# bdina9/qat-vit

Hardware: AMD Instinct MI355X
Metric: images/sec QAT student step (fwd+bwd+allreduce) (higher is better)
Workload: dtype f32 (emulated: int8 MFMA for grid x grid products; forward float operands as fp16 hi+lo pairs; backward gradients as ONE fp16 plane scaled per tensor - 2^-12 per element, <= 4e-4 relative L2 per stage against the fp32 reference, bf16-pair fallback on overflow; fp32 / exact-integer accumulate)

## Files before the change

include/qatvit.h:

```cpp
#ifndef QATVIT_H
#define QATVIT_H

#include <stdint.h>

#ifdef __cplusplus
extern "C" {
#endif
#if defined(__GNUC__) || defined(__clang__)
#pragma GCC visibility push(default)
#endif

#define QATVIT_ABI_VERSION 4

int qatvit_abi_version(void);
const char* qatvit_last_error(void);
const char* qatvit_target_arch(void);

int64_t qatvit_fq_workspace_bytes(int64_t channels);
int qatvit_fq_forward(const float* x, float* y, uint8_t* mask_bits,
                      float* running_min, float* running_max, float* scale, int32_t* zero_point,
                      const int64_t* observer_on, const int64_t* fake_quant_on,
                      float averaging_const, int32_t qmin, int32_t qmax,
                      int64_t channels, int64_t inner, int32_t per_channel, int32_t symmetric,
                      void* workspace, void* stream);
// ... 6 lines not shown
                       const float* rstd, float* dx, float* dgamma, float* dbeta,
                       int64_t rows, int64_t dim, void* stream);

int qatvit_kd_ce_loss(const float* student, const float* teacher, const int64_t* labels,
                      int64_t batch, int64_t classes, float kd_temp, float kd_alpha,
                      float label_smoothing, float* out3, float* dlogits, void* stream);

int qatvit_kd_ce_loss_table(const float* student, const float* table, int64_t table_rows,
                            const int64_t* index, const int64_t* labels, int64_t batch,
                            int64_t classes, float kd_temp, float kd_alpha, float label_smoothing,
                            float* out3, float* dlogits, void* stream);


int qatvit_gemm_nt(const void* A_hi, const void* A_lo, const void* B, float* C, int32_t M, int32_t N, int32_t K,
                   int32_t lda, int32_t ldb, int32_t ldc, const float* s1, const float* s2, const float* col_scale,
                   const float* bias, uint32_t* stats, void* stream);

int qatvit_gemm_nt_f16(const void* A16_hi, const void* A16_lo, const void* B16, float* C, int32_t M, int32_t N, int32_t K, int32_t lda, int32_t ldb,
                       int32_t ldc, const float* s1, const float* s2, const float* col_scale, const float* bias, uint32_t* stats, void* stream);

int qatvit_gemm_nt_i8_minmax(const void* A8, const void* B8, const int32_t* wsum, const float* a_qp, int32_t center, int32_t M, int32_t N, int32_t K,
                             int32_t lda, int32_t ldb, const float* s1, const float* s2, const float* col_scale, const float* bias, uint32_t* stats,
                             void* stream);

int qatvit_w8_fragment_order(const void* B8, void* B8f, int32_t N, int32_t K, void* stream);

int qatvit_i8_strip(int32_t mode, const void* A8, const void* B8f, const int32_t* wsum, const float* a_qp, int32_t center, int32_t M, int32_t N, int32_t K,
                    int32_t lda, const float* s1, const float* s2, const float* col_scale, const float* bias, uint32_t* stats, const float* out_qp,
                    int32_t qmin, int32_t qmax, void* out8, void* out8_mask, int32_t code_T, uint32_t* lut_out, uint32_t* lutq_out,
                    float* out16_scale, void* stream);

int qatvit_ln_apply_quant8(const float* x, const float* mean, const float* rstd, const float* gamma, const float* beta, const float* qp, int32_t qmin, int32_t qmax,
                           void* out8, int32_t center, int64_t M, int32_t D, void* stream);

int qatvit_i8_strip_ln(const float* x, const float* mean, const float* rstd, const float* gamma, const float* beta, int32_t ln_qmin, int32_t ln_qmax, void* out8,
                       const void* B8f, const int32_t* wsum, const float* a_qp, int32_t center, int32_t M, int32_t N, int32_t K, int32_t lda, const float* s2,
                       const float* col_scale, const float* bias, uint32_t* stats, void* stream);

int qatvit_gemm_nt_codes(const void* A8, const uint32_t* lut, const void* B16, float* C, int32_t M, int32_t N, int32_t K, int32_t lda, int32_t ldb,
                         int32_t ldc, const float* s1, const float* s2, const float* col_scale, const float* bias, uint32_t* stats, void* stream);

int qatvit_gemm_nt_i8(const void* A8, const void* B8, const int32_t* wsum, const float* a_qp, int32_t center, float* C, int32_t M,
                      int32_t N, int32_t K, int32_t lda, int32_t ldb, int32_t ldc, const float* s1, const float* s2,
                      const float* col_scale, const float* bias, uint32_t* stats, void* stream);

int64_t qatvit_gemm_tn_scratch_bytes(void);
int qatvit_gemm_tn_codes(const void* P_hi, const void* P_lo, const void* Qc, const uint32_t* lutQ, float* C, int32_t M, int32_t N, int32_t Kw, int32_t ldp,
                         int32_t ldq, int32_t ldc, const float* s1, const float* W, const float* w_scale, const int32_t* w_zp, int32_t w_per_channel,
                         int32_t w_qmin, int32_t w_qmax, float* dbias, const float* row_div, float* scratch, int64_t scratch_bytes, void* stream);
int qatvit_gemm_tn(const void* P_hi, const void* P_lo, const void* Q_hi, const void* Q_lo, float* C, int32_t M, int32_t N,
                   int32_t Kw, int32_t ldp, int32_t ldq, int32_t ldc, const float* s1, const float* W, const float* w_scale,
                   const int32_t* w_zp, int32_t w_per_channel, int32_t w_qmin, int32_t w_qmax, float* dbias,
                   const float* row_div, float* scratch, int64_t scratch_bytes, void* stream);

int qatvit_gemm_nt_dy16(const void* A16, const void* B16, float* C, int32_t M, int32_t N, int32_t K, int32_t lda, int32_t ldb, int32_t ldc, const float* s1,
                        const float* s2, void* stream);
int qatvit_gemm_tn_dy16(const void* P16, const void* Q_hi, const void* Q_lo, const void* Qc, const uint32_t* lutQ16, float* C, int32_t M, int32_t N, int32_t Kw,
                        int32_t ldp, int32_t ldq, int32_t ldc, const float* s1, const float* s2, const float* W, const float* w_scale, const int32_t* w_zp,
                        int32_t w_per_channel, int32_t w_qmin, int32_t w_qmax, float* dbias, const float* row_div, float* scratch, int64_t scratch_bytes,
                        void* stream);
int qatvit_gemm_tn_q8_dy16(const void* P16, const void* Q8, const float* a_qp, int32_t center, float* C, int32_t M, int32_t N, int32_t Kw, int32_t ldp, int32_t ldq,
                           int32_t ldc, const float* s2, const float* W, const float* w_scale, const int32_t* w_zp, int32_t w_per_channel, int32_t w_qmin,
                           int32_t w_qmax, float* dbias, const float* row_div, float* scratch, int64_t scratch_bytes, void* stream);

struct qatvit_tn_item {
    const void* P; const void* Q; const uint32_t* lut; const float* s1; const float* s2; float* C; const float* W; const float* w_scale; const int32_t* w_zp; float* dbias;
// ... 129 lines not shown
```

qat-vit_amd/csrc/capi.hip:

```cpp
#include <stdarg.h>
#include <stdlib.h>
#include <string.h>

#include "../../include/qatvit.h"
#include "qv_common.h"
#include "qv_kernels.h"

namespace qv {
static thread_local char g_err[512] = "";
void set_error(const char* fmt, ...) {
    va_list ap;
    va_start(ap, fmt);
    vsnprintf(g_err, sizeof(g_err), fmt, ap);
    va_end(ap);
}

static bool knob(const char* name) {
    const char* v = getenv(name);
    return !v || atoi(v) != 0;
}
const Knobs& knobs() {
    static const Knobs k{knob("QATVIT_I8"), knob("QATVIT_F16"), knob("QATVIT_FC2_CODES"), knob("QATVIT_FC1_BITS"), knob("QATVIT_FC2W_CODES"),
                         knob("QATVIT_WBATCH"), knob("QATVIT_ATTN_CODES"), knob("QATVIT_QKV_2PASS"), knob("QATVIT_LNB_FUSE"), knob("QATVIT_QP_LATE"),
                         knob("QATVIT_TN_STREAM"), knob("QATVIT_TN_Q8"), knob("QATVIT_ATTN_BWD_FUSED"), knob("QATVIT_F16_STRIP"), knob("QATVIT_I8_STRIP"), knob("QATVIT_LN_STRIP")};
// ... 112 lines not shown
    if (launch_w8_fragment_order(B8, B8f, N, K, (hipStream_t)stream)) return 1;
    QV_CHECK_LAUNCH("qatvit_w8_fragment_order");
    return 0;
}

int qatvit_i8_strip(int32_t mode, const void* A8, const void* B8f, const int32_t* wsum, const float* a_qp, int32_t center, int32_t M, int32_t N, int32_t K,
                    int32_t lda, const float* s1, const float* s2, const float* col_scale, const float* bias, uint32_t* stats, const float* out_qp,
                    int32_t qmin, int32_t qmax, void* out8, void* out8_mask, int32_t code_T, uint32_t* lut_out, uint32_t* lutq_out,
                    float* out16_scale, void* stream) {
    QV_CHECK_ARG(A8 && B8f && wsum && a_qp && s1, "qatvit_i8_strip: null pointer argument");
    QV_CHECK_ARG(mode == 3 || mode == 4 || mode == 7, "qatvit_i8_strip: mode %d (3 = statistics, 7 = qkv codes, 4 = fc1 codes)", mode);
    NTPost post{};
    post.mode = mode;
    post.qp = out_qp; post.qmin = qmin; post.qmax = qmax; post.out8 = out8; post.out8_mask = out8_mask; post.code_T = code_T; post.code_hd = 64;
    post.lut_out = lut_out; post.lutq_out = lutq_out; post.out16_scale = out16_scale;
    if (!launch_i8_strip(A8, B8f, wsum, a_qp, center, M, N, K, lda, N, s1, s2, col_scale, bias, stats, 1, (hipStream_t)stream, &post, true)) {
        set_error("qatvit_i8_strip: unsupported arguments (mode %d M=%d N=%d K=%d lda=%d: need K = 384 with N %% 1152 == 0 or N %% 1536 == 0, or K = 768 with "
                  "N = 2304 or 3072; lda %% 16 == 0, M < 2^22, the mode's output pointers, qmax - qmin < 256; mode 7: (N / 3) %% 384 == 0, 0 < code_T < 1024)",
                  mode, M, N, K, lda);
        return 1;
    }
    QV_CHECK_LAUNCH("qatvit_i8_strip");
    return 0;
}

int qatvit_ln_apply_quant8(const float* x, const float* mean, const float* rstd, const float* gamma, const float* beta, const float* qp, int32_t qmin, int32_t qmax,
                           void* out8, int32_t center, int64_t M, int32_t D, void* stream) {
    QV_CHECK_ARG(x && mean && rstd && gamma && beta && qp && out8, "qatvit_ln_apply_quant8: null pointer argument");
    QV_CHECK_ARG(M >= 1 && D >= 4 && D % 4 == 0, "qatvit_ln_apply_quant8: M=%lld D=%d (D %% 4 == 0)", (long long)M, D);
    if (launch_ln_apply_quant(x, mean, rstd, gamma, beta, qp, qmin, qmax, nullptr, M, D, (hipStream_t)stream, out8, center)) return 1;
    QV_CHECK_LAUNCH("qatvit_ln_apply_quant8");
    return 0;
}

int qatvit_i8_strip_ln(const float* x, const float* mean, const float* rstd, const float* gamma, const float* beta, int32_t ln_qmin, int32_t ln_qmax, void* out8,
                       const void* B8f, const int32_t* wsum, const float* a_qp, int32_t center, int32_t M, int32_t N, int32_t K, int32_t lda, const float* s2,
                       const float* col_scale, const float* bias, uint32_t* stats, void* stream) {
    QV_CHECK_ARG(x && mean && rstd && gamma && beta && out8 && B8f && wsum && a_qp && stats, "qatvit_i8_strip_ln: null pointer argument");
    if (!launch_i8_strip_ln(x, mean, rstd, gamma, beta, ln_qmin, ln_qmax, out8, B8f, wsum, a_qp, center, M, N, K, lda, s2, col_scale, bias, stats, 1,
                            (hipStream_t)stream, true)) {
        set_error("qatvit_i8_strip_ln: unsupported arguments (M=%d N=%d K=%d lda=%d: need K = 384 with N = 1152 or 1536, or K = 768 with N = 2304 or 3072; "
                  "lda %% 16 == 0, lda >= K, 0 < M < 2^22)", M, N, K, lda);
        return 1;
    }
    QV_CHECK_LAUNCH("qatvit_i8_strip_ln");
    return 0;
}

int qatvit_gemm_nt_codes(const void* A8, const uint32_t* lut, const void* B16, float* C, int32_t M, int32_t N, int32_t K, int32_t lda, int32_t ldb,
                         int32_t ldc, const float* s1, const float* s2, const float* col_scale, const float* bias, uint32_t* stats, void* stream) {
    QV_CHECK_ARG(A8 && lut && B16 && C, "qatvit_gemm_nt_codes: null pointer argument");
    if (launch_gemm_nt_codes(A8, lut, B16, C, M, N, K, lda, ldb, ldc, s1, s2, col_scale, bias, stats, 1, (hipStream_t)stream)) return 1;
    QV_CHECK_LAUNCH("qatvit_gemm_nt_codes");
    return 0;
}

int qatvit_gemm_nt_i8(const void* A8, const void* B8, const int32_t* wsum, const float* a_qp, int32_t center, float* C, int32_t M, int32_t N,
                      int32_t K, int32_t lda, int32_t ldb, int32_t ldc, const float* s1, const float* s2, const float* col_scale, const float* bias,
                      uint32_t* stats, void* stream) {
    QV_CHECK_ARG(A8 && B8 && wsum && a_qp && C, "qatvit_gemm_nt_i8: null pointer argument");
    if (launch_gemm_nt_i8(A8, B8, wsum, a_qp, center, C, M, N, K, lda, ldb, ldc, s1, s2, col_scale, bias, stats, 1, (hipStream_t)stream)) return 1;
    QV_CHECK_LAUNCH("qatvit_gemm_nt_i8");
    return 0;
}

int qatvit_gemm_tn(const void* P_hi, const void* P_lo, const void* Q_hi, const void* Q_lo, float* C, int32_t M, int32_t N, int32_t Kw, int32_t ldp,
// ... 153 lines not shown
```

qat-vit_amd/csrc/elt.hip:

```cpp
#include <stdlib.h>

#include "qv_common.h"
#include "qv_device.h"
#include "qv_kernels.h"
#include "qv_qparams.h"

namespace qv {

struct QP { float s, inv, zp, on; };
__device__ inline QP load_qp(const float* qp) { return QP{qp[0], qp[1], qp[2], qp[3]}; }
__device__ inline float fqv(float x, const QP& q, float fqmin, float fqmax, bool& in) {
    const float t = rintf(x * q.inv) + q.zp;
    in = (t >= fqmin && t <= fqmax) || q.on == 0.f;
    const float y = (fminf(fmaxf(t, fqmin), fqmax) - q.zp) * q.s;
    return q.on != 0.f ? y : x;
}
__device__ inline float fqi(float x, const QP& q, float fqmin, float fqmax) {
    return fminf(fmaxf(rintf(x * q.inv) + q.zp, fqmin), fqmax) - q.zp;
}

__device__ inline void store_split4(__bf16* hi, __bf16* lo, int64_t off, float a, float b, float c, float d) {
    uint2 h, l;
    split_pair(a, b, h.x, l.x);
    split_pair(c, d, h.y, l.y);
// ... 106 lines not shown
            if (act[j]) s += (v[j].x + v[j].y) + (v[j].z + v[j].w);
        }
#pragma unroll
        for (int j = 0; j < NV; ++j)
            if (MODE != 2 && act[j]) *reinterpret_cast<float4*>(x_new + row * D + cc[j]) = v[j];
        const float mu = wave_sum(s) / (float)D;
        float qq = 0.f;
#pragma unroll
        for (int j = 0; j < NV; ++j) {
            v[j].x -= mu; v[j].y -= mu; v[j].z -= mu; v[j].w -= mu;
            if (act[j]) qq += (v[j].x * v[j].x + v[j].y * v[j].y) + (v[j].z * v[j].z + v[j].w * v[j].w);
        }
        const float rs = rsqrtf(wave_sum(qq) / (float)D + eps);
        if (lane == 0) { mean[row] = mu; rstd[row] = rs; }
        if (MODE == 1 && maskbits && lane < 4) {
#pragma unroll
            for (int j = 0; j < NV; ++j)
                maskbits[(row * NV + j) * 4 + lane] = lane == 0 ? mb[j][0] : lane == 1 ? mb[j][1] : lane == 2 ? mb[j][2] : mb[j][3];
        }
#pragma unroll
        for (int j = 0; j < NV; ++j) {
            if (act[j]) {
                const float o0 = v[j].x * rs * g[j].x + bb[j].x, o1 = v[j].y * rs * g[j].y + bb[j].y, o2 = v[j].z * rs * g[j].z + bb[j].z,
                            o3 = v[j].w * rs * g[j].w + bb[j].w;
                mn = fminf(fminf(mn, o0), fminf(o1, fminf(o2, o3)));
                mx = fmaxf(fmaxf(mx, o0), fmaxf(o1, fmaxf(o2, o3)));
            }
        }
    }
    mn = wave_min(mn);
    mx = wave_max(mx);
    __shared__ float smn[4], smx[4];
    if (lane == 0) { smn[threadIdx.x >> 6] = mn; smx[threadIdx.x >> 6] = mx; }
    __syncthreads();
    const float bmn = fminf(fminf(smn[0], smn[1]), fminf(smn[2], smn[3])), bmx = fmaxf(fmaxf(smx[0], smx[1]), fmaxf(smx[2], smx[3]));
    if (threadIdx.x == 0) stat_atomic(stats, stat_slots, bmn, bmx);
}

__global__ __launch_bounds__(256) void k_ln_apply_quant(const float* __restrict__ x, const float* __restrict__ mean, const float* __restrict__ rstd,
                                                        const float* __restrict__ gamma, const float* __restrict__ beta, const float* __restrict__ qp,
                                                        int qmin, int qmax, __bf16* __restrict__ out, int64_t M, int D,
                                                        int8_t* __restrict__ out8, int center, int out_f16, const QpLate late) {
    __shared__ float sQp[4];
    QP q;
    if (late.stats) { const float4 r = qp_late_resolve(late, sQp); q = QP{r.x, r.y, r.z, r.w}; }
    else q = load_qp(qp);
    const int d4 = D / 4;
    const int64_t n4 = M * d4;
    for (int64_t i = blockIdx.x * (int64_t)blockDim.x + threadIdx.x; i < n4; i += (int64_t)gridDim.x * blockDim.x) {
        const int64_t row = i / d4;
        const int c = (int)(i % d4) * 4;
        const float mu = mean[row], rs = rstd[row];
        const float4 v = *reinterpret_cast<const float4*>(x + row * D + c);
        const float4 g = *reinterpret_cast<const float4*>(gamma + c), b = *reinterpret_cast<const float4*>(beta + c);
        bf16x4 o;
        o[0] = (__bf16)fqi((v.x - mu) * rs * g.x + b.x, q, qmin, qmax);
        o[1] = (__bf16)fqi((v.y - mu) * rs * g.y + b.y, q, qmin, qmax);
        o[2] = (__bf16)fqi((v.z - mu) * rs * g.z + b.z, q, qmin, qmax);
        o[3] = (__bf16)fqi((v.w - mu) * rs * g.w + b.w, q, qmin, qmax);
        if (out && out_f16) *reinterpret_cast<uint2*>(out + row * D + c) = make_uint2(pk_f16((float)o[0], (float)o[1]), pk_f16((float)o[2], (float)o[3]));
        else if (out) *reinterpret_cast<bf16x4*>(out + row * D + c) = o;
        if (out8) {
            const float sh = q.zp - (float)center;
            char4 o8 = make_char4((signed char)((float)o[0] + sh), (signed char)((float)o[1] + sh), (signed char)((float)o[2] + sh),
                                  (signed char)((float)o[3] + sh));
            *reinterpret_cast<char4*>(out8 + row * D + c) = o8;
// ... 392 lines not shown
__global__ __launch_bounds__(256) void k_wquant(const float* __restrict__ W, const float* __restrict__ qp, int per_channel, int qmin, int qmax,
                                                __bf16* __restrict__ wq, __bf16* __restrict__ wqT, int N, int K) {
    wquant_body(W, qp, per_channel, qmin, qmax, wq, wqT, N, K, blockIdx.x, blockIdx.y);
}
__global__ __launch_bounds__(256) void k_w_quant_all(const WQuantTab t) {
    int wi = 0;
    while (wi + 1 < t.n && (int)blockIdx.x >= t.blk0[wi + 1]) ++wi;
    const int b = blockIdx.x - t.blk0[wi], kt = (t.K[wi] + 31) / 32;
    wquant_body(t.W[wi], t.qp[wi], t.per_channel, t.qmin, t.qmax, reinterpret_cast<__bf16*>(t.wq[wi]), reinterpret_cast<__bf16*>(t.wqT[wi]), t.N[wi],
                t.K[wi], b % kt, b / kt, reinterpret_cast<int8_t*>(t.w8[wi]), t.wsum[wi], reinterpret_cast<_Float16*>(t.w16[wi]),
                reinterpret_cast<int8_t*>(t.w8f[wi]), t.wT16 ? wT16_gap_bytes(t.N[wi], t.K[wi]) : 0, ((t.wT16f_mask >> wi) & 1ull) != 0);
}
static_assert(sizeof(WQuantTab) <= 4096, "WQuantTab travels as a kernel argument");
__global__ __launch_bounds__(256) void k_w8_fragment_order(const int8_t* __restrict__ B8, int8_t* __restrict__ B8f, int N, int K) {
    const int64_t i = blockIdx.x * (int64_t)blockDim.x + threadIdx.x;
    if (i >= (int64_t)N * K) return;
    B8f[w8f_offset((int)(i / K), (int)(i % K), K)] = B8[i];
}
int launch_w8_fragment_order(const void* B8, void* B8f, int N, int K, hipStream_t st) {
    if (N < 48 || N % 48 != 0 || K % 64 != 0 || !B8 || !B8f) { set_error("w8_fragment_order: need N %% 48 == 0, K %% 64 == 0 (N=%d K=%d)", N, K); return 1; }
    k_w8_fragment_order<<<cdiv((int64_t)N * K, 256), 256, 0, st>>>(reinterpret_cast<const int8_t*>(B8), reinterpret_cast<int8_t*>(B8f), N, K);
    return 0;
}

int launch_img_patches(const float* img, void* out_bf16, const float* qp, int qmin, int qmax, int B, int C, int H, int W, int P, hipStream_t st,
                       void* out8, int center) {
    if (P % 8 != 0 || H % P != 0 || W % P != 0) { set_error("img_patches: patch %d must be a multiple of 8 and divide %dx%d", P, H, W); return 1; }
    const int64_t n8 = (int64_t)B * C * H * W / 8;
    k_img_patches<<<flat_grid(n8), 256, 0, st>>>(img, reinterpret_cast<__bf16*>(out_bf16), qp, qmin, qmax, B, C, H, W, P, reinterpret_cast<int8_t*>(out8),
                                                 center);
    return 0;
}

int launch_resid_fq_lnstats(int mode, const float* x_prev, const float* Y, const float* qpY, int qmin, int qmax, const float* cls, const float* pos,
                            float* x_new, float* mean, float* rstd, const float* gamma, const float* beta, float eps, uint32_t* stats, int stat_slots,
                            int64_t M, int D, int T, hipStream_t st, void* maskbits, const QpLate* late) {
    if (D % 4 != 0 || D > 256 * kMaxV) { set_error("resid_fq_lnstats: D=%d unsupported (need D%%4==0, D<=768)", D); return 1; }
    unsigned long long* mbits = mode != 1 ? nullptr : reinterpret_cast<unsigned long long*>(maskbits);
    const QpLate lt = late ? *late : QpLate{};
#define QV_RESID(MODE_, NV_) k_resid_fq_lnstats<MODE_, NV_><<<rows_grid(M), 256, 0, st>>>(x_prev, Y, qpY, qmin, qmax, cls, pos, x_new, mean, rstd, gamma, beta, eps, stats, stat_slots, M, D, T, mbits, lt)
    const int nv = (D + 255) / 256;
    if (mode == 0) { if (nv == 1) QV_RESID(0, 1); else if (nv == 2) QV_RESID(0, 2); else QV_RESID(0, 3); }
    else if (mode == 1) { if (nv == 1) QV_RESID(1, 1); else if (nv == 2) QV_RESID(1, 2); else QV_RESID(1, 3); }
    else { if (nv == 1) QV_RESID(2, 1); else if (nv == 2) QV_RESID(2, 2); else QV_RESID(2, 3); }
#undef QV_RESID
    return 0;
}

int launch_ln_apply_quant(const float* x, const float* mean, const float* rstd, const float* gamma, const float* beta, const float* qp, int qmin,
                          int qmax, void* out_bf16, int64_t M, int D, hipStream_t st, void* out8, int center, bool out_f16, const QpLate* late) {
    k_ln_apply_quant<<<flat_grid(M * (D / 4)), 256, 0, st>>>(x, mean, rstd, gamma, beta, qp, qmin, qmax, reinterpret_cast<__bf16*>(out_bf16), M, D,
                                                             reinterpret_cast<int8_t*>(out8), center, out_f16 ? 1 : 0, late ? *late : QpLate{});
    return 0;
}

int launch_ln_quant8(const float* x, const float* gamma, const float* beta, float eps, const float* qp, int qmin, int qmax, int center, void* out8,
                     float* mean, float* rstd, int64_t nrows, int64_t row_stride, int D, hipStream_t st) {
    if (D % 4 != 0 || D > 256 * kMaxV) { set_error("ln_quant8: D=%d unsupported (need D%%4==0, D<=768)", D); return 1; }
    const int nv = (D + 255) / 256, grid = rows_grid(nrows);
    int8_t* o = reinterpret_cast<int8_t*>(out8);
    if (nv == 1) k_ln_quant8<1><<<grid, 256, 0, st>>>(x, gamma, beta, eps, qp, qmin, qmax, center, o, mean, rstd, nrows, row_stride, D);
    else if (nv == 2) k_ln_quant8<2><<<grid, 256, 0, st>>>(x, gamma, beta, eps, qp, qmin, qmax, center, o, mean, rstd, nrows, row_stride, D);
    else k_ln_quant8<3><<<grid, 256, 0, st>>>(x, gamma, beta, eps, qp, qmin, qmax, center, o, mean, rstd, nrows, row_stride, D);
    return 0;
}
int launch_cls_rows(const float* cls, const float* pos, float* x, int B, int T, int D, hipStream_t st) {
    k_cls_rows<<<cdiv((int64_t)B * D, 256), 256, 0, st>>>(cls, pos, x, B, T, D);
    return 0;
}

int launch_mask_bwd(int gelu_bwd, const float* d, const float* Y, const float* qp, int qmin, int qmax, const float* col_scale, int ncols,
                    void* dst_hi, void* dst_lo, int64_t n, hipStream_t st, const float* o16_mul, uint32_t* o16_amax) {
    __bf16* h = reinterpret_cast<__bf16*>(dst_hi);
    __bf16* l = reinterpret_cast<__bf16*>(dst_lo);
// ... 92 lines not shown
```

qat-vit_amd/csrc/qv_kernels.h:

```cpp
#pragma once
#include <hip/hip_runtime.h>
#include <stdint.h>

namespace qv {

int launch_fq_forward(const float* x, float* y, uint8_t* mask_bits, float* running_min, float* running_max, float* scale,
                      int32_t* zero_point, const int64_t* observer_on, const int64_t* fake_quant_on, float c, int qmin, int qmax,
                      int64_t channels, int64_t inner, bool per_channel, bool symmetric, void* workspace, hipStream_t st);
int launch_fq_backward(const float* dy, const uint8_t* mask_bits, float* dx, int64_t n, hipStream_t st);

int launch_ln_forward(const float* x, const float* gamma, const float* beta, float* y, float* mean, float* rstd, int64_t rows,
                      int64_t dim, float eps, hipStream_t st);
int launch_ln_backward(const float* dy, const float* x, const float* gamma, const float* mean, const float* rstd, float* dx,
                       float* dgamma, float* dbeta, int64_t rows, int64_t dim, hipStream_t st);

int launch_kd_ce_loss(const float* student, const float* teacher, const int64_t* labels, int64_t batch, int64_t classes, float kd_temp,
                      float kd_alpha, float label_smoothing, float* out3, float* dlogits, hipStream_t st);
int launch_kd_ce_loss_table(const float* student, const float* table, int64_t table_rows, const int64_t* index, const int64_t* labels, int64_t batch,
                            int64_t classes, float kd_temp, float kd_alpha, float label_smoothing, float* out3, float* dlogits, hipStream_t st);

int launch_minmax(const float* x, int64_t channels, int64_t inner, int per_channel, uint32_t* ws, int nslots, hipStream_t st);
int launch_ws_init(uint32_t* ws, int64_t slots, hipStream_t st);
int launch_qparams(uint32_t* ws, float* running_min, float* running_max, float* scale, int32_t* zero_point, const int64_t* observer_on,
                   const int64_t* fake_quant_on, float c, int qmin, int qmax, int64_t channels, int symmetric, float* qp_out, int reset_ws,
// ... 72 lines not shown
    const int cg = n / 48, cr = n % 48, j = cr / 16, r = cr % 16, kt = k / 64, kk = k % 64;
    return ((((int64_t)cg * (K / 64) + kt) * 3 + j) * 64 + (kk / 16) * 16 + r) * 16 + (kk % 16);
}
int launch_w8_fragment_order(const void* B8, void* B8f, int N, int K, hipStream_t st);
int launch_gemm_nt_codes(const void* A8, const uint32_t* lut, const void* B16, float* C, int M, int N, int K, int lda, int ldb, int ldc, const float* s1,
                         const float* s2, const float* col_scale, const float* bias, uint32_t* stats, int stat_slots, hipStream_t st, const NTPost* post = nullptr);
constexpr int64_t kTnScratchBytes = 256ll * 128 * 384 * 4;
int launch_gemm_tn(const void* P_hi, const void* P_lo, const void* Q_hi, const void* Q_lo, float* C, int M, int N, int Kw, int ldp, int ldq, int ldc,
                   const float* s1, const float* W, const float* w_scale, const int32_t* w_zp, int w_per_channel, int w_qmin, int w_qmax,
                   float* dbias, const float* row_div, hipStream_t st, float* partial = nullptr, int64_t partial_bytes = 0);
int launch_gemm_tn_codes(const void* P_hi, const void* P_lo, const void* Qc, const uint32_t* lutQ, float* C, int M, int N, int Kw, int ldp, int ldq, int ldc,
                         const float* s1, const float* W, const float* w_scale, const int32_t* w_zp, int w_per_channel, int w_qmin, int w_qmax, float* dbias,
                         const float* row_div, hipStream_t st, float* partial = nullptr, int64_t partial_bytes = 0);
int launch_gemm_tn_dy16(const void* P16, const void* Q_hi, const void* Q_lo, float* C, int M, int N, int Kw, int ldp, int ldq, int ldc, const float* s1,
                        const float* s2, const float* W, const float* w_scale, const int32_t* w_zp, int w_per_channel, int w_qmin, int w_qmax, float* dbias,
                        const float* row_div, hipStream_t st, float* partial = nullptr, int64_t partial_bytes = 0, bool bf16 = false);
int launch_gemm_tn_codes_dy16(const void* P16, const void* Qc, const uint32_t* lutQ16, float* C, int M, int N, int Kw, int ldp, int ldq, int ldc, const float* s1,
                              const float* s2, const float* W, const float* w_scale, const int32_t* w_zp, int w_per_channel, int w_qmin, int w_qmax, float* dbias,
                              const float* row_div, hipStream_t st, float* partial = nullptr, int64_t partial_bytes = 0);
int launch_gemm_tn_q8_dy16(const void* P16, const void* Q8, const float* a_qp, int center, float* C, int M, int N, int Kw, int ldp, int ldq, int ldc, const float* s2,
                           const float* W, const float* w_scale, const int32_t* w_zp, int w_per_channel, int w_qmin, int w_qmax, float* dbias, const float* row_div,
                           hipStream_t st, float* partial = nullptr, int64_t partial_bytes = 0);
struct TNStreamGemm {
    const void* P; const void* Q; const uint32_t* lut; const float* s1; const float* s2; float* C; const float* W; const float* w_scale; const int32_t* w_zp; float* dbias;
    const float* row_div; int N, Kw, ldp, ldq, ldc;
};
int64_t tn_stream_scratch_bytes();
int launch_tn_stream(int mode, const TNStreamGemm* items, int n, int M, int center, int w_per_channel, int w_qmin, int w_qmax, float* partial, int64_t partial_bytes,
                     hipStream_t st);
int launch_img_patches(const float* img, void* out_bf16, const float* qp, int qmin, int qmax, int B, int C, int H, int W, int P, hipStream_t st,
                       void* out8 = nullptr, int center = 0);
int launch_resid_fq_lnstats(int mode, const float* x_prev, const float* Y, const float* qpY, int qmin, int qmax, const float* cls, const float* pos,
                            float* x_new, float* mean, float* rstd, const float* gamma, const float* beta, float eps, uint32_t* stats, int stat_slots,
                            int64_t M, int D, int T, hipStream_t st, void* maskbits = nullptr, const QpLate* late = nullptr);
inline int64_t ln_maskbits_bytes(int64_t M, int D) { return M * ((D + 255) / 256) * 32; }
struct LnBwdNext { const void* maskbits; const float* colscale; void* out_hi; void* out_lo; const float* o16_mul = nullptr; uint32_t* o16_amax = nullptr; };
int launch_ln_apply_quant(const float* x, const float* mean, const float* rstd, const float* gamma, const float* beta, const float* qp, int qmin,
                          int qmax, void* out_bf16, int64_t M, int D, hipStream_t st, void* out8 = nullptr, int center = 0,
                          bool out_f16 = false,
                          const QpLate* late = nullptr);
int launch_ln_quant8(const float* x, const float* gamma, const float* beta, float eps, const float* qp, int qmin, int qmax, int center, void* out8,
                     float* mean, float* rstd, int64_t nrows, int64_t row_stride, int D, hipStream_t st);
int launch_cls_rows(const float* cls, const float* pos, float* x, int B, int T, int D, hipStream_t st);
int launch_mask_bwd(int gelu_bwd, const float* d, const float* Y, const float* qp, int qmin, int qmax, const float* col_scale, int ncols,
                    void* dst_hi, void* dst_lo, int64_t n, hipStream_t st, const float* o16_mul = nullptr, uint32_t* o16_amax = nullptr);
int launch_ln_bwd_fq(int acc, const float* dH, const float* x, const float* mean, const float* rstd, const float* gamma, const float* beta,
                     const float* qp, int qmin, int qmax, const float* dx_in, float* dx_out, float* dgamma, float* dbeta, int64_t M, int D, int T,
                     int cls_only, hipStream_t st, const LnBwdNext* next = nullptr);
int launch_head_fwd(const float* x, const float* mean, const float* rstd, const float* gamma, const float* beta, const float* qp_norm, int qmin,
                    int qmax, const void* wq, const float* w_scale, int w_per_channel, const float* bias, float* hq, float* logits_pre,
                    uint32_t* stats, int stat_slots, int B, int D, int T, int C, hipStream_t st);
int launch_logits_fq(const float* pre, const float* qp, int qmin, int qmax, float* out, int n, hipStream_t st);
int launch_head_bwd(const float* dlogits, const float* logits_pre, const float* qp_logits, int qmin, int qmax, const float* hq, const float* qp_norm,
                    const void* wq, const float* W, const float* w_scale, const int32_t* w_zp, int w_per_channel, int w_qmin, int w_qmax, float* dW,
                    float* dbias, float* dh, int B, int D, int C, hipStream_t st);
int launch_embed_bwd(const float* dx0, const float* Y0, const float* qp, int qmin, int qmax, float* dpos, float* dcls, void* dY0_hi, void* dY0_lo,
                     int B, int T, int D, hipStream_t st);
constexpr int kMaxW = 52;
struct WObsTab { const float* W[kMaxW]; uint32_t* ws[kMaxW]; int N[kMaxW], K[kMaxW], blk0[kMaxW + 1]; int n, per_channel, nslots; };
struct WQpTab {
    uint32_t* ws[kMaxW]; float* rmin[kMaxW]; float* rmax[kMaxW]; float* scale[kMaxW]; int32_t* zp[kMaxW]; float* qp[kMaxW];
    const int64_t* obs_on[kMaxW]; const int64_t* fq_on[kMaxW]; int N[kMaxW], blk0[kMaxW + 1]; int n, per_channel, nslots, qmin, qmax; float c;
};
struct WQuantTab {
    const float* W[kMaxW]; const float* qp[kMaxW]; void* wq[kMaxW]; void* wqT[kMaxW]; void* w8[kMaxW]; int32_t* wsum[kMaxW];
    void* w16[kMaxW];
    void* w8f[kMaxW];
// ... 81 lines not shown
```

qat-vit_amd/native.py:

```python
from __future__ import annotations

import ctypes
import os
import subprocess
from ctypes import c_char_p, c_double, c_float, c_int, c_int32, c_int64, c_void_p

_HERE = os.path.dirname(os.path.abspath(__file__))
LIB_PATH = os.path.join(_HERE, "libqatvit.so")
CSRC = os.path.join(_HERE, "csrc")
_lib = None

SIGNATURES = {
    "qatvit_abi_version": (c_int, []),
    "qatvit_last_error": (c_char_p, []),
    "qatvit_target_arch": (c_char_p, []),
    "qatvit_fq_workspace_bytes": (c_int64, [c_int64]),
    "qatvit_fq_forward": (c_int, [c_void_p] * 9 + [c_float, c_int32, c_int32, c_int64, c_int64, c_int32, c_int32, c_void_p, c_void_p]),
    "qatvit_fq_backward": (c_int, [c_void_p, c_void_p, c_void_p, c_int64, c_void_p]),
    "qatvit_ln_forward": (c_int, [c_void_p] * 6 + [c_int64, c_int64, c_float, c_void_p]),
    "qatvit_ln_backward": (c_int, [c_void_p] * 8 + [c_int64, c_int64, c_void_p]),
    "qatvit_kd_ce_loss": (c_int, [c_void_p, c_void_p, c_void_p, c_int64, c_int64, c_float, c_float, c_float, c_void_p, c_void_p, c_void_p]),
    "qatvit_kd_ce_loss_table": (c_int, [c_void_p, c_void_p, c_int64, c_void_p, c_void_p, c_int64, c_int64, c_float, c_float, c_float, c_void_p, c_void_p, c_void_p]),
    "qatvit_optim_grad_norm": (c_int, [c_void_p] * 4 + [c_int32, c_int64, c_float, c_void_p, c_void_p, c_void_p]),
    "qatvit_optim_adamw": (c_int, [c_void_p] * 7 + [c_int32, c_int64] + [c_double] * 5 + [c_int64, c_void_p, c_void_p]),
    "qatvit_gemm_nt": (c_int, [c_void_p] * 4 + [c_int32] * 6 + [c_void_p] * 6),
    "qatvit_gemm_nt_f16": (c_int, [c_void_p] * 4 + [c_int32] * 6 + [c_void_p] * 6),
    "qatvit_gemm_nt_i8_minmax": (c_int, [c_void_p] * 4 + [c_int32] * 6 + [c_void_p] * 6),
    "qatvit_w8_fragment_order": (c_int, [c_void_p, c_void_p, c_int32, c_int32, c_void_p]),
    "qatvit_i8_strip": (c_int, [c_int32] + [c_void_p] * 4 + [c_int32] * 5 + [c_void_p] * 6 + [c_int32, c_int32, c_void_p, c_void_p, c_int32] + [c_void_p] * 4),
    "qatvit_ln_apply_quant8": (c_int, [c_void_p] * 6 + [c_int32, c_int32, c_void_p, c_int32, c_int64, c_int32, c_void_p]),
    "qatvit_i8_strip_ln": (c_int, [c_void_p] * 5 + [c_int32, c_int32] + [c_void_p] * 4 + [c_int32] * 5 + [c_void_p] * 5),
    "qatvit_gemm_nt_codes": (c_int, [c_void_p] * 4 + [c_int32] * 6 + [c_void_p] * 6),
    "qatvit_gemm_nt_i8": (c_int, [c_void_p] * 4 + [c_int32, c_void_p] + [c_int32] * 6 + [c_void_p] * 6),
    "qatvit_gemm_tn_scratch_bytes": (c_int64, []),
    "qatvit_gemm_tn": (c_int, [c_void_p] * 5 + [c_int32] * 6 + [c_void_p] * 4 + [c_int32] * 3 + [c_void_p] * 3 + [c_int64, c_void_p]),
    "qatvit_gemm_tn_codes": (c_int, [c_void_p] * 5 + [c_int32] * 6 + [c_void_p] * 4 + [c_int32] * 3 + [c_void_p] * 3 + [c_int64, c_void_p]),
    "qatvit_gemm_nt_dy16": (c_int, [c_void_p] * 3 + [c_int32] * 6 + [c_void_p] * 3),
    "qatvit_gemm_tn_dy16": (c_int, [c_void_p] * 6 + [c_int32] * 6 + [c_void_p] * 5 + [c_int32] * 3 + [c_void_p] * 3 + [c_int64, c_void_p]),
    "qatvit_gemm_tn_q8_dy16": (c_int, [c_void_p] * 3 + [c_int32, c_void_p] + [c_int32] * 6 + [c_void_p] * 4 + [c_int32] * 3 + [c_void_p] * 3 + [c_int64, c_void_p]),
    "qatvit_gemm_tn_stream_scratch_bytes": (c_int64, []),
    "qatvit_gemm_tn_stream_dy16": (c_int, [c_int32, c_void_p, c_int32, c_int32, c_int32, c_int32, c_int32, c_int32, c_void_p, c_int64, c_void_p]),
    "qatvit_attn_padded_tokens": (c_int32, [c_int32]),
    "qatvit_attn_forward": (c_int, [c_void_p, c_void_p] + [c_int32] * 6 + [c_void_p] * 4),
    "qatvit_attn_forward_f16": (c_int, [c_void_p, c_void_p] + [c_int32] * 6 + [c_void_p] * 9),
    "qatvit_attn_backward": (c_int, [c_void_p, c_void_p] + [c_int32] * 6 + [c_void_p] * 11),
    "qatvit_student_num_params": (c_int32, [c_void_p]),
    "qatvit_student_num_act_fq": (c_int32, [c_void_p]),
    "qatvit_student_num_weight_fq": (c_int32, [c_void_p]),
    "qatvit_student_workspace_bytes": (c_int64, [c_void_p]),
    "qatvit_student_init": (c_int, [c_void_p, c_void_p, c_void_p]),
    "qatvit_student_forward": (c_int, [c_void_p] * 8),
    "qatvit_student_backward": (c_int, [c_void_p] * 7 + [c_int32, c_int32, c_void_p]),
    "qatvit_student_forward_stages": (c_int, [c_void_p] * 7 + [c_int32, c_int32, c_int32, c_void_p]),
    "qatvit_student_forward_part": (c_int, [c_void_p] * 5 + [c_int32, c_int32, c_int32, c_void_p]),
    "qatvit_student_backward_stages": (c_int, [c_void_p] * 7 + [c_int32, c_int32, c_int32, c_void_p]),
    "qatvit_student_tensor_offset": (c_int64, [c_void_p, c_char_p, c_int32]),
    "qatvit_student_dy16_supported": (c_int32, [c_void_p]),
    "qatvit_student_ln_in_strip": (c_int32, [c_void_p, c_int32]),
    "qatvit_student_dy16_to_pair": (c_int, [c_void_p, c_void_p, c_void_p]),
    "qatvit_student_dy16_set_mirror": (c_int, [c_void_p, c_void_p, c_void_p, c_void_p]),
    "qatvit_teacher_workspace_bytes": (c_int64, [c_void_p]),
    "qatvit_teacher_forward": (c_int, [c_void_p] * 8),
    "qatvit_teacher_forward_f16": (c_int, [c_void_p, c_void_p, c_void_p, c_int32, c_void_p, c_void_p, c_void_p, c_void_p]),
# ... 22 lines not shown
    "qatvit_image_batch": (c_int, [c_void_p, c_void_p] + [c_int32] * 4 + [c_void_p] * 4),
    "qatvit_eval_accumulate": (c_int, [c_void_p, c_int32, c_int64, c_void_p, c_int64, c_int64, c_void_p, c_int64, c_void_p, c_int64, c_void_p, c_void_p, c_void_p]),
    "qatvit_profile_start": (c_int, [c_void_p, c_int32, c_int32]),
    "qatvit_profile_stop": (c_int, [c_void_p, c_void_p, c_void_p, c_void_p]),
}


class Cfg(ctypes.Structure):
    _fields_ = [(n, c_int32) for n in ("batch", "img_size", "patch_size", "in_chans", "embed_dim", "depth", "num_heads", "mlp_hidden",
                                       "num_classes", "act_qmin", "act_qmax", "w_qmin", "w_qmax", "w_per_channel")] + \
               [("averaging_const", c_float), ("ln_eps", c_float)]


def vit_params(model) -> list:
    pe = model.patch_embed.proj
    ps = [pe.weight, pe.bias, model.cls_token, model.pos_embed]
    for b in model.blocks:
        ps += [b.norm1.weight, b.norm1.bias, b.attn.qkv.weight, b.attn.qkv.bias, b.attn.proj.weight, b.attn.proj.bias,
               b.norm2.weight, b.norm2.bias, b.mlp.fc1.weight, b.mlp.fc1.bias, b.mlp.fc2.weight, b.mlp.fc2.bias]
    return ps + [model.norm.weight, model.norm.bias, model.head.weight, model.head.bias]


def vit_shape(model) -> dict:
    b0 = model.blocks[0]
    return dict(img_size=model.patch_embed.img_size, patch_size=model.patch_embed.patch_size, in_chans=model.patch_embed.proj.weight.shape[1],
                embed_dim=model.embed_dim, depth=len(model.blocks), num_heads=b0.attn.num_heads, mlp_hidden=b0.mlp.fc1.weight.shape[0],
                num_classes=model.head.weight.shape[0], ln_eps=float(b0.norm1.eps))


class TNItem(ctypes.Structure):
    _fields_ = [(n, c_void_p) for n in ("P", "Q", "lut", "s1", "s2", "C", "W", "w_scale", "w_zp", "dbias", "row_div")] + [(n, c_int32) for n in ("N", "Kw", "ldp", "ldq", "ldc")]


class FQ(ctypes.Structure):
    _fields_ = [(n, c_void_p) for n in ("min_val", "max_val", "scale", "zero_point", "observer_on", "fake_quant_on")]


def build(verbose: bool = False) -> str:
    r = subprocess.run(["make", "-C", CSRC, "-j8"], capture_output=True, text=True)
    if r.returncode != 0:
        raise RuntimeError("building libqatvit.so failed:\n" + r.stdout[-4000:] + r.stderr[-4000:])
    if verbose:
        print(r.stdout[-2000:])
    return LIB_PATH


def lib() -> ctypes.CDLL:
    global _lib
    if _lib is None:
        if not os.path.exists(LIB_PATH):
            raise RuntimeError(
                f"{LIB_PATH} is missing: the MI355X path has no fallback. Build it with "
                "`python -c 'import __graft_entry__ as g; g.build()'` (needs hipcc)."
            )
        L = ctypes.CDLL(LIB_PATH)
        for name, (res, args) in SIGNATURES.items():
            fn = getattr(L, name)
            fn.restype, fn.argtypes = res, args
        if L.qatvit_abi_version() != 4:
            raise RuntimeError("libqatvit.so ABI version mismatch")
        _lib = L
    return _lib


def check(status: int, what: str) -> None:
    if status != 0:
# ... 34 lines not shown
```

Measured before the change: 16360.

## Add persistent double-buffered streaming kernel for residual fake-quant plus LayerNorm stats

Adds a persistent-grid, wave-per-row kernel for mode 1 of the residual + fake-quant + LayerNorm-stats fusion. It double-buffers raw buffer loads of x_prev and Y for the next row while computing the current one, and hoists gamma/beta and the qparams out of the row loop. The aim is to hide memory latency and cut per-block setup on this bandwidth-bound pass. It also exposes a C API, a reference-form toggle and a grid override, which adds API surface and another code path to keep numerically consistent.

```diff
diff --git a/include/qatvit.h b/include/qatvit.h
--- a/include/qatvit.h
+++ b/include/qatvit.h
@@ -62,6 +62,22 @@
 
 int qatvit_ln_apply_quant8(const float* x, const float* mean, const float* rstd, const float* gamma, const float* beta, const float* qp, int32_t qmin, int32_t qmax,
                            void* out8, int32_t center, int64_t M, int32_t D, void* stream);
+
+typedef struct qatvit_qp_late {
+    const uint32_t* stats;
+    const float* min_val; const float* max_val; const float* scale; const int32_t* zero_point;
+    const int64_t* observer_on; const int64_t* fake_quant_on;
+    float averaging_const; int32_t qmin, qmax;
+    float* qp_out;
+    float* staged;
+} qatvit_qp_late;
+int qatvit_resid_fq_lnstats(int32_t mode, const float* x_prev, const float* Y, const float* qpY, int32_t qmin, int32_t qmax, const float* cls, const float* pos,
+                            float* x_new, float* mean, float* rstd, const float* gamma, const float* beta, float eps, uint32_t* stats, int32_t stat_slots,
+                            int64_t M, int32_t D, int32_t T, void* maskbits, const qatvit_qp_late* late, int32_t grid, void* stream);
+int qatvit_resid_fq_lnstats_ref(int32_t mode, const float* x_prev, const float* Y, const float* qpY, int32_t qmin, int32_t qmax, const float* cls, const float* pos,
+                                float* x_new, float* mean, float* rstd, const float* gamma, const float* beta, float eps, uint32_t* stats, int32_t stat_slots,
+                                int64_t M, int32_t D, int32_t T, void* maskbits, const qatvit_qp_late* late, int32_t grid, void* stream);
+int qatvit_resid_ref_form(int32_t on);
 
 int qatvit_i8_strip_ln(const float* x, const float* mean, const float* rstd, const float* gamma, const float* beta, int32_t ln_qmin, int32_t ln_qmax, void* out8,
                        const void* B8f, const int32_t* wsum, const float* a_qp, int32_t center, int32_t M, int32_t N, int32_t K, int32_t lda, const float* s2,
diff --git a/qat-vit_amd/csrc/capi.hip b/qat-vit_amd/csrc/capi.hip
--- a/qat-vit_amd/csrc/capi.hip
+++ b/qat-vit_amd/csrc/capi.hip
@@ -168,6 +168,41 @@
     QV_CHECK_LAUNCH("qatvit_ln_apply_quant8");
     return 0;
 }
+
+static int resid_capi(const char* who, bool ref_form, int32_t mode, const float* x_prev, const float* Y, const float* qpY, int32_t qmin, int32_t qmax, const float* cls,
+                      const float* pos, float* x_new, float* mean, float* rstd, const float* gamma, const float* beta, float eps, uint32_t* stats,
+                      int32_t stat_slots, int64_t M, int32_t D, int32_t T, void* maskbits, const qatvit_qp_late* late, int32_t grid, void* stream) {
+    QV_CHECK_ARG(mode >= 0 && mode <= 2, "%s: mode %d", who, mode);
+    QV_CHECK_ARG(mean && rstd && gamma && beta && stats && (mode == 2 || x_new) && (mode == 0 ? cls && pos && Y : x_prev && (mode == 2 || Y)),
+                 "%s: null pointer argument", who);
+    QV_CHECK_ARG(late || qpY, "%s: neither qpY nor late", who);
+    QV_CHECK_ARG(M >= 1 && D >= 4 && T >= 1 && (stat_slots == 1 || stat_slots == kStatSlots), "%s: M=%lld D=%d T=%d stat_slots=%d", who, (long long)M, D, T, stat_slots);
+    QpLate L{};
+    if (late) {
+        QV_CHECK_ARG(late->stats && late->min_val && late->max_val && late->scale && late->zero_point && late->observer_on && late->fake_quant_on && late->qp_out &&
+                         late->staged, "%s: null pointer in late", who);
+        L = QpLate{late->stats, late->min_val, late->max_val, late->scale, late->zero_point, late->observer_on, late->fake_quant_on, late->averaging_const,
+                   late->qmin, late->qmax, late->qp_out, late->staged};
+    }
+    if (launch_resid_fq_lnstats(mode, x_prev, Y, qpY ? qpY : (late ? late->qp_out : nullptr), qmin, qmax, cls, pos, x_new, mean, rstd, gamma, beta, eps, stats, stat_slots, M, D,
+                                T, (hipStream_t)stream, maskbits, late ? &L : nullptr, ref_form, grid))
+        return 1;
+    QV_CHECK_LAUNCH(who);
+    return 0;
+}
+int qatvit_resid_fq_lnstats(int32_t mode, const float* x_prev, const float* Y, const float* qpY, int32_t qmin, int32_t qmax, const float* cls, const float* pos,
+                            float* x_new, float* mean, float* rstd, const float* gamma, const float* beta, float eps, uint32_t* stats, int32_t stat_slots,
+                            int64_t M, int32_t D, int32_t T, void* maskbits, const qatvit_qp_late* late, int32_t grid, void* stream) {
+    return resid_capi("qatvit_resid_fq_lnstats", false, mode, x_prev, Y, qpY, qmin, qmax, cls, pos, x_new, mean, rstd, gamma, beta, eps, stats, stat_slots, M, D, T,
+                      maskbits, late, grid, stream);
+}
+int qatvit_resid_fq_lnstats_ref(int32_t mode, const float* x_prev, const float* Y, const float* qpY, int32_t qmin, int32_t qmax, const float* cls, const float* pos,
+                                float* x_new, float* mean, float* rstd, const float* gamma, const float* beta, float eps, uint32_t* stats, int32_t stat_slots,
+                                int64_t M, int32_t D, int32_t T, void* maskbits, const qatvit_qp_late* late, int32_t grid, void* stream) {
+    return resid_capi("qatvit_resid_fq_lnstats_ref", true, mode, x_prev, Y, qpY, qmin, qmax, cls, pos, x_new, mean, rstd, gamma, beta, eps, stats, stat_slots, M, D, T,
+                      maskbits, late, grid, stream);
+}
+int qatvit_resid_ref_form(int32_t on) { return resid_ref_form(on) ? 1 : 0; }
 
 int qatvit_i8_strip_ln(const float* x, const float* mean, const float* rstd, const float* gamma, const float* beta, int32_t ln_qmin, int32_t ln_qmax, void* out8,
                        const void* B8f, const int32_t* wsum, const float* a_qp, int32_t center, int32_t M, int32_t N, int32_t K, int32_t lda, const float* s2,
diff --git a/qat-vit_amd/csrc/elt.hip b/qat-vit_amd/csrc/elt.hip
--- a/qat-vit_amd/csrc/elt.hip
+++ b/qat-vit_amd/csrc/elt.hip
@@ -162,6 +162,106 @@
     mx = wave_max(mx);
     __shared__ float smn[4], smx[4];
     if (lane == 0) { smn[threadIdx.x >> 6] = mn; smx[threadIdx.x >> 6] = mx; }
+    __syncthreads();
+    const float bmn = fminf(fminf(smn[0], smn[1]), fminf(smn[2], smn[3])), bmx = fmaxf(fmaxf(smx[0], smx[1]), fmaxf(smx[2], smx[3]));
+    if (threadIdx.x == 0) stat_atomic(stats, stat_slots, bmn, bmx);
+}
+
+typedef uint32_t u32x2 __attribute__((ext_vector_type(2)));
+__device__ inline void pin4u(u32x4& v) { asm volatile("" : "+v"(v)); }
+template <int NV>
+__global__ __launch_bounds__(256) void k_resid_fq_lnstats_stream(const float* __restrict__ x_prev, const float* __restrict__ Y, const float* __restrict__ qpY,
+                                                                 int qmin, int qmax, float* __restrict__ x_new, float* __restrict__ mean,
+                                                                 float* __restrict__ rstd, const float* __restrict__ gamma, const float* __restrict__ beta,
+                                                                 float eps, uint32_t* __restrict__ stats, int stat_slots, int64_t M, int D,
+                                                                 unsigned long long* __restrict__ maskbits, const QpLate late) {
+    __shared__ float sQp[4];
+    const int lane = threadIdx.x & 63;
+    const int wave = __builtin_amdgcn_readfirstlane(threadIdx.x >> 6);
+    const int64_t stride = (int64_t)gridDim.x * 4;
+    int64_t row = (int64_t)blockIdx.x * 4 + wave;
+    auto issue = [&](int64_t r, u32x4 (&b)[NV], u32x4 (&y)[NV]) {
+        const int64_t ext = r < M ? (int64_t)D * 4 : 0;
+        const auto rb = make_rsrc(x_prev + r * D, ext), ry = make_rsrc(Y + r * D, ext);
+#pragma unroll
+        for (int j = 0; j < NV; ++j) {
+            b[j] = __builtin_amdgcn_raw_buffer_load_b128(rb, lane * 16 + 1024 * j, 0, 0);
+            y[j] = __builtin_amdgcn_raw_buffer_load_b128(ry, lane * 16 + 1024 * j, 0, 0);
+        }
+    };
+    u32x4 bA[NV], yA[NV], bB[NV], yB[NV];
+    issue(row, bA, yA);
+    bool act[NV];
+    float4 g[NV], bb[NV];
+#pragma unroll
+    for (int j = 0; j < NV; ++j) {
+        const int c = lane * 4 + 256 * j;
+        act[j] = c < D;
+        g[j] = *reinterpret_cast<const float4*>(gamma + (act[j] ? c : 0));
+        bb[j] = *reinterpret_cast<const float4*>(beta + (act[j] ? c : 0));
+    }
+    QP q;
+    if (late.stats) { const float4 r = qp_late_resolve(late, sQp); q = QP{r.x, r.y, r.z, r.w}; }
+    else q = load_qp(qpY);
+#pragma unroll
+    for (int j = 0; j < NV; ++j) { pin4(g[j]); pin4(bb[j]); pin4u(bA[j]); pin4u(yA[j]); }
+    float mn = INFINITY, mx = -INFINITY;
+    auto body = [&](int64_t r, const u32x4 (&b)[NV], const u32x4 (&yy)[NV]) {
+        float4 v[NV];
+        float s = 0.f;
+        unsigned long long mb[NV][4];
+#pragma unroll
+        for (int j = 0; j < NV; ++j) {
+            const float4 base = __builtin_bit_cast(float4, b[j]), yr = __builtin_bit_cast(float4, yy[j]);
+            bool i0, i1, i2, i3;
+            const float4 y = make_float4(fqv(yr.x, q, qmin, qmax, i0), fqv(yr.y, q, qmin, qmax, i1), fqv(yr.z, q, qmin, qmax, i2), fqv(yr.w, q, qmin, qmax, i3));
+            mb[j][0] = __ballot(act[j] && i0); mb[j][1] = __ballot(act[j] && i1);
+            mb[j][2] = __ballot(act[j] && i2); mb[j][3] = __ballot(act[j] && i3);
+            v[j] = make_float4(base.x + y.x, base.y + y.y, base.z + y.z, base.w + y.w);
+            if (act[j]) s += (v[j].x + v[j].y) + (v[j].z + v[j].w);
+        }
+        const auto rx = make_rsrc(x_new + r * D, (int64_t)D * 4);
+#pragma unroll
+        for (int j = 0; j < NV; ++j) __builtin_amdgcn_raw_buffer_store_b128(__builtin_bit_cast(u32x4, v[j]), rx, lane * 16 + 1024 * j, 0, 0);
+        const float mu = wave_sum(s) / (float)D;
+        float qq = 0.f;
+#pragma unroll
+        for (int j = 0; j < NV; ++j) {
+            v[j].x -= mu; v[j].y -= mu; v[j].z -= mu; v[j].w -= mu;
+            if (act[j]) qq += (v[j].x * v[j].x + v[j].y * v[j].y) + (v[j].z * v[j].z + v[j].w * v[j].w);
+        }
+        const float rs = rsqrtf(wave_sum(qq) / (float)D + eps);
+        __builtin_amdgcn_raw_buffer_store_b32(__builtin_bit_cast(uint32_t, mu), make_rsrc(mean + r, 4), lane * 4, 0, 0);
+        __builtin_amdgcn_raw_buffer_store_b32(__builtin_bit_cast(uint32_t, rs), make_rsrc(rstd + r, 4), lane * 4, 0, 0);
+        unsigned long long w = mb[0][0];
+#pragma unroll
+        for (int j = 0; j < NV; ++j)
+#pragma unroll
+            for (int e = 0; e < 4; ++e)
+                if (lane == j * 4 + e) w = mb[j][e];
+        __builtin_amdgcn_raw_buffer_store_b64(__builtin_bit_cast(u32x2, w), make_rsrc(maskbits + r * (NV * 4), maskbits ? NV * 32 : 0), lane * 8, 0, 0);
+#pragma unroll
+        for (int j = 0; j < NV; ++j) {
+            if (act[j]) {
+                const float o0 = v[j].x * rs * g[j].x + bb[j].x, o1 = v[j].y * rs * g[j].y + bb[j].y, o2 = v[j].z * rs * g[j].z + bb[j].z,
+                            o3 = v[j].w * rs * g[j].w + bb[j].w;
+                mn = fminf(fminf(mn, o0), fminf(o1, fminf(o2, o3)));
+                mx = fmaxf(fmaxf(mx, o0), fmaxf(o1, fmaxf(o2, o3)));
+            }
+        }
+    };
+    while (row < M) {
+        issue(row + stride, bB, yB);
+        body(row, bA, yA);
+        if (row + stride >= M) break;
+        issue(row + 2 * stride, bA, yA);
+        body(row + stride, bB, yB);
+        row += 2 * stride;
+    }
+    mn = wave_min(mn);
+    mx = wave_max(mx);
+    __shared__ float smn[4], smx[4];
+    if (lane == 0) { smn[wave] = mn; smx[wave] = mx; }
     __syncthreads();
     const float bmn = fminf(fminf(smn[0], smn[1]), fminf(smn[2], smn[3])), bmx = fmaxf(fmaxf(smx[0], smx[1]), fmaxf(smx[2], smx[3]));
     if (threadIdx.x == 0) stat_atomic(stats, stat_slots, bmn, bmx);
@@ -620,14 +720,31 @@
     return 0;
 }
 
+static bool g_resid_ref_form = false;
+bool resid_ref_form(int on) {
+    const bool was = g_resid_ref_form;
+    if (on >= 0) g_resid_ref_form = on != 0;
+    return was;
+}
+static inline int resid_stream_grid(int64_t rows) {
+    int64_t b = (rows + 7) / 8;
+    return (int)(b < 1 ? 1 : (b > 8192 ? 8192 : b));
+}
 int launch_resid_fq_lnstats(int mode, const float* x_prev, const float* Y, const float* qpY, int qmin, int qmax, const float* cls, const float* pos,
                             float* x_new, float* mean, float* rstd, const float* gamma, const float* beta, float eps, uint32_t* stats, int stat_slots,
-                            int64_t M, int D, int T, hipStream_t st, void* maskbits, const QpLate* late) {
+                            int64_t M, int D, int T, hipStream_t st, void* maskbits, const QpLate* late, bool ref_form, int grid) {
     if (D % 4 != 0 || D > 256 * kMaxV) { set_error("resid_fq_lnstats: D=%d unsupported (need D%%4==0, D<=768)", D); return 1; }
+    if (grid < 0 || grid > 65535) { set_error("resid_fq_lnstats: grid=%d", grid); return 1; }
     unsigned long long* mbits = mode != 1 ? nullptr : reinterpret_cast<unsigned long long*>(maskbits);
     const QpLate lt = late ? *late : QpLate{};
-#define QV_RESID(MODE_, NV_) k_resid_fq_lnstats<MODE_, NV_><<<rows_grid(M), 256, 0, st>>>(x_prev, Y, qpY, qmin, qmax, cls, pos, x_new, mean, rstd, gamma, beta, eps, stats, stat_slots, M, D, T, mbits, lt)
     const int nv = (D + 255) / 256;
+    if (mode == 1 && !ref_form && !g_resid_ref_form) {
+#define QV_RESID_STREAM(NV_) k_resid_fq_lnstats_stream<NV_><<<grid ? grid : resid_stream_grid(M), 256, 0, st>>>(x_prev, Y, qpY, qmin, qmax, x_new, mean, rstd, gamma, beta, eps, stats, stat_slots, M, D, mbits, lt)
+        if (nv == 1) QV_RESID_STREAM(1); else if (nv == 2) QV_RESID_STREAM(2); else QV_RESID_STREAM(3);
+#undef QV_RESID_STREAM
+        return 0;
+    }
+#define QV_RESID(MODE_, NV_) k_resid_fq_lnstats<MODE_, NV_><<<grid ? grid : rows_grid(M), 256, 0, st>>>(x_prev, Y, qpY, qmin, qmax, cls, pos, x_new, mean, rstd, gamma, beta, eps, stats, stat_slots, M, D, T, mbits, lt)
     if (mode == 0) { if (nv == 1) QV_RESID(0, 1); else if (nv == 2) QV_RESID(0, 2); else QV_RESID(0, 3); }
     else if (mode == 1) { if (nv == 1) QV_RESID(1, 1); else if (nv == 2) QV_RESID(1, 2); else QV_RESID(1, 3); }
     else { if (nv == 1) QV_RESID(2, 1); else if (nv == 2) QV_RESID(2, 2); else QV_RESID(2, 3); }
diff --git a/qat-vit_amd/csrc/qv_kernels.h b/qat-vit_amd/csrc/qv_kernels.h
--- a/qat-vit_amd/csrc/qv_kernels.h
+++ b/qat-vit_amd/csrc/qv_kernels.h
@@ -128,7 +128,9 @@
                        void* out8 = nullptr, int center = 0);
 int launch_resid_fq_lnstats(int mode, const float* x_prev, const float* Y, const float* qpY, int qmin, int qmax, const float* cls, const float* pos,
                             float* x_new, float* mean, float* rstd, const float* gamma, const float* beta, float eps, uint32_t* stats, int stat_slots,
-                            int64_t M, int D, int T, hipStream_t st, void* maskbits = nullptr, const QpLate* late = nullptr);
+                            int64_t M, int D, int T, hipStream_t st, void* maskbits = nullptr, const QpLate* late = nullptr,
+                            bool ref_form = false, int grid = 0);
+bool resid_ref_form(int on);
 inline int64_t ln_maskbits_bytes(int64_t M, int D) { return M * ((D + 255) / 256) * 32; }
 struct LnBwdNext { const void* maskbits; const float* colscale; void* out_hi; void* out_lo; const float* o16_mul = nullptr; uint32_t* o16_amax = nullptr; };
 int launch_ln_apply_quant(const float* x, const float* mean, const float* rstd, const float* gamma, const float* beta, const float* qp, int qmin,
diff --git a/qat-vit_amd/native.py b/qat-vit_amd/native.py
--- a/qat-vit_amd/native.py
+++ b/qat-vit_amd/native.py
@@ -29,6 +29,9 @@
     "qatvit_w8_fragment_order": (c_int, [c_void_p, c_void_p, c_int32, c_int32, c_void_p]),
     "qatvit_i8_strip": (c_int, [c_int32] + [c_void_p] * 4 + [c_int32] * 5 + [c_void_p] * 6 + [c_int32, c_int32, c_void_p, c_void_p, c_int32] + [c_void_p] * 4),
     "qatvit_ln_apply_quant8": (c_int, [c_void_p] * 6 + [c_int32, c_int32, c_void_p, c_int32, c_int64, c_int32, c_void_p]),
+    "qatvit_resid_fq_lnstats": (c_int, [c_int32] + [c_void_p] * 3 + [c_int32, c_int32] + [c_void_p] * 7 + [c_float, c_void_p, c_int32, c_int64, c_int32, c_int32, c_void_p, c_void_p, c_int32, c_void_p]),
+    "qatvit_resid_fq_lnstats_ref": (c_int, [c_int32] + [c_void_p] * 3 + [c_int32, c_int32] + [c_void_p] * 7 + [c_float, c_void_p, c_int32, c_int64, c_int32, c_int32, c_void_p, c_void_p, c_int32, c_void_p]),
+    "qatvit_resid_ref_form": (c_int, [c_int32]),
     "qatvit_i8_strip_ln": (c_int, [c_void_p] * 5 + [c_int32, c_int32] + [c_void_p] * 4 + [c_int32] * 5 + [c_void_p] * 5),
     "qatvit_gemm_nt_codes": (c_int, [c_void_p] * 4 + [c_int32] * 6 + [c_void_p] * 6),
     "qatvit_gemm_nt_i8": (c_int, [c_void_p] * 4 + [c_int32, c_void_p] + [c_int32] * 6 + [c_void_p] * 6),
@@ -117,6 +120,11 @@
     _fields_ = [(n, c_void_p) for n in ("P", "Q", "lut", "s1", "s2", "C", "W", "w_scale", "w_zp", "dbias", "row_div")] + [(n, c_int32) for n in ("N", "Kw", "ldp", "ldq", "ldc")]
 
 
+class QpLate(ctypes.Structure):
+    _fields_ = [(n, c_void_p) for n in ("stats", "min_val", "max_val", "scale", "zero_point", "observer_on", "fake_quant_on")] + \
+               [("averaging_const", c_float), ("qmin", c_int32), ("qmax", c_int32), ("qp_out", c_void_p), ("staged", c_void_p)]
+
+
 class FQ(ctypes.Structure):
     _fields_ = [(n, c_void_p) for n in ("min_val", "max_val", "scale", "zero_point", "observer_on", "fake_quant_on")]
 
```

New measurement: 16480, median of 6. Within noise of the previous version (+0.8%).
